# bayesiains/nflows

Measured on AMD Instinct MI355X. Metric: log_prob samples/sec (dim=64, K=8, 32-layer RQ-NSF) + max |fwd∘inv − x|, higher is better.
Workload: dtype f32 (inputs, outputs, spline arithmetic, accumulation; conditioner GEMMs: every fp32 operand carried as 3 f16 pieces = 33 significand bits, i.e. at the reference's own fp32 operand width, 5 cross products per multiply-add -- 3 on the f16 MFMA, the 2 at the 2^-22 level from the pieces' high bytes on

## Files before the change

### include/nflows_amd.h

```cpp
#ifndef NFLOWS_AMD_H
#define NFLOWS_AMD_H

#include <stddef.h>
#include <stdint.h>

#ifdef __cplusplus
extern "C" {
#endif

#define NFA_ABI_VERSION 16

#define NFA_OK 0
#define NFA_ERR_INVALID_ARGUMENT 1
#define NFA_ERR_UNSUPPORTED 2
#define NFA_ERR_MIN_BIN_WIDTH 3
#define NFA_ERR_MIN_BIN_HEIGHT 4
#define NFA_ERR_HIP 5

#define NFA_STATUS_OUTSIDE_DOMAIN 1
#define NFA_STATUS_NEG_DISCRIMINANT 2
#define NFA_STATUS_BAD_INDEX 4

#define NFA_FLAG_INVERSE 1
#define NFA_FLAG_ACCUMULATE_LOGABSDET 2
// ... 307 lines not shown
                                   const nfa_rqs_spec *spec, int32_t inverse, void *stream);
int nfa_quadratic_spline_backward_f32(const float *inputs, const float *unnormalized_widths,
                                      const float *unnormalized_heights, int32_t num_heights,
                                      const float *grad_outputs, const float *grad_logabsdet,
                                      float *grad_inputs, float *grad_unnormalized_widths,
                                      float *grad_unnormalized_heights, int64_t n,
                                      const nfa_rqs_spec *spec, int32_t inverse, void *stream);

int nfa_cubic_spline_backward_f32(const float *inputs, const float *unnormalized_widths,
                                  const float *unnormalized_heights,
                                  const float *unnorm_derivatives_left,
                                  const float *unnorm_derivatives_right, const float *grad_outputs,
                                  const float *grad_logabsdet, float *grad_inputs,
                                  float *grad_unnormalized_widths, float *grad_unnormalized_heights,
                                  float *grad_unnorm_derivatives_left,
                                  float *grad_unnorm_derivatives_right, int64_t n,
                                  const nfa_rqs_spec *spec, int32_t inverse, void *stream);

size_t nfa_linear_wgrad_workspace_bytes(int64_t batch, int32_t in_features, int32_t out_features);
int nfa_linear_wgrad_f32(const float *inputs, const float *grad_outputs, float *grad_weight,
                         float *grad_bias, void *workspace, int64_t batch, int32_t in_features,
                         int32_t out_features, int32_t flags, void *stream);

size_t nfa_linear_wgrad_batched_workspace_bytes(int32_t count, int64_t batch, int32_t in_features, int32_t out_features);
int nfa_linear_wgrad_batched_f32(int32_t count, const float *const *inputs, const float *const *grad_outputs,
                                 float *const *grad_weight, float *const *grad_bias, void *workspace, int64_t batch,
                                 int32_t in_features, int32_t out_features, int32_t flags, void *stream);

int nfa_profile_enable(int32_t max_launches);
int nfa_profile_collect(float *durations_ms, int32_t capacity, int32_t *count);

int nfa_last_layer_kernel(char *buffer, int32_t capacity);

void nfa_debug_k7_trace(void *device_buffer);

#ifdef __cplusplus
}
#endif
#endif
```

### nflows_amd/_native.py

```python
import ctypes
import os

import torch

_PKG_DIR = os.path.dirname(os.path.abspath(__file__))
LIB_PATH = os.environ.get("NFLOWS_AMD_LIB") or os.path.join(_PKG_DIR, "libnflows_amd.so")

OK = 0
ERR_INVALID_ARGUMENT = 1
ERR_UNSUPPORTED = 2
ERR_MIN_BIN_WIDTH = 3
ERR_MIN_BIN_HEIGHT = 4
ERR_HIP = 5

STATUS_OUTSIDE_DOMAIN = 1
STATUS_NEG_DISCRIMINANT = 2
STATUS_BAD_INDEX = 4

FLAG_INVERSE, FLAG_ACCUMULATE_LOGABSDET, FLAG_WEIGHTS_BF16X3, FLAG_LOGITS_LOG2E = 1, 2, 4, 8
FLAG_STANDARD_NORMAL_LOG_PROB, FLAG_SKIP_OUTPUTS = 16, 32
FLAG_RESIDUAL_BLOCKS = 64
FLAG_PAD_COLUMNS_SHIFT = 8
FLAG_ACTIVATION_SHIFT = 12
ACTIVATION_RELU, ACTIVATION_LEAKY_RELU, ACTIVATION_ELU, ACTIVATION_TANH = 0, 1, 2, 3
# ... 36 lines not shown
    "nfa_rqs_flow_resnet_context_redo_f32",
    "nfa_linear_spline_f32",
    "nfa_quadratic_spline_f32",
    "nfa_cubic_spline_f32",
    "nfa_linear_spline_backward_f32",
    "nfa_quadratic_spline_backward_f32",
    "nfa_cubic_spline_backward_f32",
    "nfa_rqs_elementwise_f32",
    "nfa_searchsorted_f32",
    "nfa_rqs_shared_f32",
    "nfa_affine_coupling_f32",
    "nfa_affine_autoregressive_f32",
    "nfa_permute_cols_b32",
    "nfa_lu_linear_f32",
    "nfa_lu_linear_backward_f32",
    "nfa_norm_workspace_bytes",
    "nfa_norm_slab_count",
    "nfa_norm_column_stats_f32",
    "nfa_norm_column_sums_f32",
    "nfa_norm_map_f32",
    "nfa_norm_map_backward_f32",
    "nfa_norm_batch_backward_f32",
    "nfa_rowsum_f32",
    "nfa_standard_normal_log_prob_f32",
    "nfa_sum_count_f64",
    "nfa_sum_count_workspace_bytes",
    "nfa_linear_wgrad_workspace_bytes",
    "nfa_linear_wgrad_f32",
    "nfa_linear_wgrad_batched_workspace_bytes",
    "nfa_linear_wgrad_batched_f32",
    "nfa_profile_enable",
    "nfa_profile_collect",
    "nfa_last_layer_kernel",
    "nfa_debug_k7_trace",
)


class NativeLibraryMissing(RuntimeError):
    pass


class NativeError(RuntimeError):
    def __init__(self, code, message):
        super().__init__("libnflows_amd: %s (code %d)" % (message, code))
        self.code = code


class RqsSpec(ctypes.Structure):

    _fields_ = [
        ("num_bins", ctypes.c_int32),
        ("tails", ctypes.c_int32),
        ("left", ctypes.c_double),
        ("right", ctypes.c_double),
        ("bottom", ctypes.c_double),
        ("top", ctypes.c_double),
        ("min_bin_width", ctypes.c_double),
        ("min_bin_height", ctypes.c_double),
        ("min_derivative", ctypes.c_double),
        ("softplus_beta", ctypes.c_double),
        ("tail_logit", ctypes.c_double),
        ("wh_divisor", ctypes.c_double),
    ]


_lib = None
# ... 101 lines not shown
    lib.nfa_norm_slab_count.argtypes = [i64, i32]
    lib.nfa_norm_column_stats_f32.restype = ctypes.c_int
    lib.nfa_norm_column_stats_f32.argtypes = [vp] * 5 + [i64, i32, vp]
    lib.nfa_norm_column_sums_f32.restype = ctypes.c_int
    lib.nfa_norm_column_sums_f32.argtypes = [vp] * 7 + [i64, i32, vp]
    lib.nfa_norm_map_f32.restype = ctypes.c_int
    lib.nfa_norm_map_f32.argtypes = [vp] * 10 + [i64, i32, ctypes.c_double, i32, i32, vp]
    lib.nfa_norm_map_backward_f32.restype = ctypes.c_int
    lib.nfa_norm_map_backward_f32.argtypes = [vp] * 9 + [i64, i32, ctypes.c_double, i32, i32, vp]
    lib.nfa_norm_batch_backward_f32.restype = ctypes.c_int
    lib.nfa_norm_batch_backward_f32.argtypes = [vp] * 7 + [i64, i32, vp]
    lib.nfa_rowsum_f32.restype = ctypes.c_int
    lib.nfa_rowsum_f32.argtypes = [vp, vp, i64, i64, vp]
    lib.nfa_standard_normal_log_prob_f32.restype = ctypes.c_int
    lib.nfa_standard_normal_log_prob_f32.argtypes = [vp, vp, vp, i64, i64, vp]
    lib.nfa_sum_count_f64.restype = ctypes.c_int
    lib.nfa_sum_count_f64.argtypes = [vp, i64, vp, vp, vp]
    lib.nfa_sum_count_workspace_bytes.restype = ctypes.c_size_t
    lib.nfa_sum_count_workspace_bytes.argtypes = []
    lib.nfa_linear_wgrad_workspace_bytes.restype = ctypes.c_size_t
    lib.nfa_linear_wgrad_workspace_bytes.argtypes = [i64, i32, i32]
    lib.nfa_linear_wgrad_f32.restype = ctypes.c_int
    lib.nfa_linear_wgrad_f32.argtypes = [vp, vp, vp, vp, vp, i64, i32, i32, i32, vp]
    lib.nfa_linear_wgrad_batched_workspace_bytes.restype = ctypes.c_size_t
    lib.nfa_linear_wgrad_batched_workspace_bytes.argtypes = [i32, i64, i32, i32]
    lib.nfa_linear_wgrad_batched_f32.restype = ctypes.c_int
    lib.nfa_linear_wgrad_batched_f32.argtypes = [i32, vp, vp, vp, vp, vp, i64, i32, i32, i32, vp]
    lib.nfa_profile_enable.restype = ctypes.c_int
    lib.nfa_profile_enable.argtypes = [i32]
    lib.nfa_profile_collect.restype = ctypes.c_int
    lib.nfa_profile_collect.argtypes = [ctypes.POINTER(ctypes.c_float), i32, ctypes.POINTER(i32)]
    lib.nfa_last_layer_kernel.restype = ctypes.c_int
    lib.nfa_last_layer_kernel.argtypes = [ctypes.c_char_p, i32]


def load():
    global _lib
    if _lib is None:
        if not os.path.exists(LIB_PATH):
            raise NativeLibraryMissing(
                "%s not found; nflows_amd has no fallback path. Build it with "
                "`make -C nflows_amd/csrc` (hipcc --offload-arch=gfx950)." % LIB_PATH
            )
        lib = ctypes.CDLL(LIB_PATH)
        missing = [name for name in EXPORTS if not hasattr(lib, name)]
        if missing:
            raise NativeLibraryMissing("%s lacks symbols: %s" % (LIB_PATH, ", ".join(missing)))
        _declare(lib)
        if lib.nfa_abi_version() != ABI_VERSION:
            raise NativeLibraryMissing("ABI version mismatch: library %d, binding %d"
                                       % (lib.nfa_abi_version(), ABI_VERSION))
        _lib = lib
    return _lib


def check(code):
    if code == OK:
        return
    lib = load()
    msg = lib.nfa_strerror(code).decode()
    if code in (ERR_MIN_BIN_WIDTH, ERR_MIN_BIN_HEIGHT):
        raise ValueError(msg)
    if code == ERR_HIP:
        msg += " (hipError_t %d)" % lib.nfa_last_hip_error()
    raise NativeError(code, msg)

# ... 31 lines not shown
```

### nflows_amd/csrc/launch_plan.hpp

```cpp
#pragma once

#include <stddef.h>
#include <stdint.h>

namespace nfa {

constexpr int kBlock = 256;
constexpr int kWave = 64;
constexpr int kDefaultDynLds = 64 * 1024;
constexpr int kCuLds = 160 * 1024;

inline int round_up4(int n) { return (n + 3) & ~3; }

inline bool aligned16(const void* p) { return (reinterpret_cast<uintptr_t>(p) & 15) == 0; }


inline int sample_rows(int lanes, int dt, int D, int64_t batch) {
    int R = dt > 0 ? lanes / dt : lanes / (D < lanes ? D : lanes);
    if (R < 1) R = 1;
    if ((int64_t)R > batch) R = (int)batch;
    return R;
}

struct SampleTile {
// ... 14 lines not shown
        t.C = (int)((budget - chunk_fixed) / ((size_t)P * 4));
        t.C = (t.C / kBlock) * kBlock;
        if (t.C >= dt) t.C = 0;
    }
    t.lds = (size_t)lds_floats(t.R, t.C) * 4;
    t.ok = t.lds <= budget && (int64_t)t.R * dt < 65536 && (int64_t)t.R * D < 65536;
    return t;
}

inline bool aligned_tile(int dt, int D, int P, int R, int64_t batch) {
    return dt > 0 && (dt * P) % 4 == 0 && D % 4 == 0 && R * dt <= kBlock && R * D <= 2 * kBlock && (int64_t)R <= batch;
}

inline int64_t full_rows(int64_t batch, int64_t rows_per_tile) { return (batch / rows_per_tile) * rows_per_tile; }

template <typename F>
inline int plan_element_tile(int floor, size_t budget, F&& bytes) {
    int T = kBlock;
    while (T > floor && (size_t)bytes(T) > budget) T >>= 1;
    return (size_t)bytes(T) <= budget ? T : 0;
}

inline int64_t persistent_grid(int cus, int per_cu, int64_t tiles) {
    const int64_t g = (int64_t)cus * per_cu;
    return g > tiles ? tiles : g;
}
inline int64_t persistent_grid(int cus, size_t lds, int cap, int64_t tiles) {
    int per_cu = (int)((size_t)kCuLds / (lds + 256));
    if (per_cu > cap) per_cu = cap;
    if (per_cu < 1) per_cu = 1;
    return persistent_grid(cus, per_cu, tiles);
}

}
```

### nflows_amd/csrc/rqs_resnet_f16x3.hip

```cpp

#include "rqs_resnet_f16x3_kernel.hpp"

using namespace nfa;

static k8x::KernelFn f16x3_kernel(bool inverse, int init_ks, int K, bool dbg) {
    if (K != 8) {
        const k8x::KernelFn kern = k8x::bins_kernel_a(K, inverse, init_ks);
        return kern ? kern : k8x::bins_kernel_b(K, inverse, init_ks);
    }
    if (init_ks == 4)
        return dbg ? (inverse ? k8x::rqs_resnet_f16x3_kernel<true, 4, true> : k8x::rqs_resnet_f16x3_kernel<false, 4, true>)
                   : (inverse ? k8x::rqs_resnet_f16x3_kernel<true, 4> : k8x::rqs_resnet_f16x3_kernel<false, 4>);
    return dbg ? (inverse ? k8x::rqs_resnet_f16x3_kernel<true, 2, true> : k8x::rqs_resnet_f16x3_kernel<false, 2, true>)
               : (inverse ? k8x::rqs_resnet_f16x3_kernel<true, 2> : k8x::rqs_resnet_f16x3_kernel<false, 2>);
}

static int launch_f16x3(const LayerCall& c, const float* scales, float act_scale, float* dbg_logits = nullptr) {
    int exponent = 0;
    if (!(act_scale > 0.0f) || frexpf(act_scale, &exponent) != 0.5f) return NFA_ERR_INVALID_ARGUMENT;
    k8x::Args a;
    int activation = 0;
    int rc = check_layer_call(c, {NFA_FLAG_ACTIVATION_MASK, true, false, false}, &a.sp, &activation);
    if (rc != NFA_OK) return rc;
    if (activation != NFA_ACTIVATION_RELU || (dbg_logits && a.sp.K != 8)) return NFA_ERR_UNSUPPORTED;
    if (c.batch == 0) return NFA_OK;
    if (!layer_buffers_given(c) || !c.bias || !scales || !c.redo) return NFA_ERR_INVALID_ARGUMENT;
    rc = fill_layer_args(a, c);
    if (rc != NFA_OK) return rc;
    a.act_scale = act_scale;
    a.bias = c.bias;
    a.scales = scales;
    a.tables = c.tables;
    a.redo = c.redo;
    a.dbg_logits = dbg_logits;
    const int init_ks = c.num_identity > 32 ? 4 : 2;
    const int rows_per_feature = spline_rows_per_feature(a.sp.K);
    a.num_stages = init_ks + 16 * c.num_blocks + 2 * (c.num_transform * rows_per_feature / 32);
    a.bias_per_layer = 128 + 256 * c.num_blocks + c.num_transform * rows_per_feature;
    const size_t lds = (size_t)kRing * kStageVec4 * 16 + (size_t)(kBlock / kWave) * c.features * kRowPad * sizeof(float) +
                       (size_t)c.num_transform * rows_per_feature * sizeof(float);
    int64_t blocks = c.batch >> 7;
    const int64_t per_cu = lds + 2048 <= 80 * 1024 ? 2 : 1;
    const int64_t cap = (int64_t)device_cu_count() * per_cu;
    if (blocks > cap) blocks = cap;
    const bool inv = (c.flags & NFA_FLAG_INVERSE) != 0;
    const k8x::KernelFn kern = f16x3_kernel(inv, init_ks, a.sp.K, dbg_logits);
    if (!kern) return NFA_ERR_UNSUPPORTED;
    note_layer_kernel("k8x::rqs_resnet_f16x3_kernel<inverse=%d, init_ks=%d, K=%d, dbg=%d>", inv ? 1 : 0, init_ks, a.sp.K, dbg_logits ? 1 : 0);
    return launch_kernel(kern, dim3((unsigned)blocks), dim3(kBlock), lds, (hipStream_t)c.stream, a, kCuLds - 2048);
}

extern "C" int nfa_rqs_flow_resnet_f16x3_f32(const float* inputs, const void* weights_packed, const float* bias_packed,
                                             const float* scales, const int32_t* flow_tables, int32_t num_layers,
                                             float* outputs, float* logabsdet, int32_t* redo_blocks, int32_t* status,
                                             int64_t batch, int32_t features, int32_t num_transform,
                                             int32_t num_identity, int32_t hidden_features, int32_t num_blocks,
                                             float act_scale, const nfa_rqs_spec* spec, int32_t flags, void* stream) {
    return launch_f16x3({inputs, weights_packed, bias_packed, flow_tables, num_layers, outputs, logabsdet, redo_blocks,
                         status, batch, features, num_transform, num_identity, hidden_features, num_blocks, spec, flags,
                         stream, nullptr, 0, 0},
                        scales, act_scale);
}

extern "C" int nfa_rqs_flow_resnet_f16x3_logits_f32(const float* inputs, const void* weights_packed,
                                                    const float* bias_packed, const float* scales,
                                                    const int32_t* flow_tables, int32_t num_layers, float* outputs,
                                                    float* logabsdet, int32_t* redo_blocks, int32_t* status,
                                                    int64_t batch, int32_t features, int32_t num_transform,
                                                    int32_t num_identity, int32_t hidden_features, int32_t num_blocks,
                                                    float act_scale, const nfa_rqs_spec* spec, int32_t flags,
                                                    void* stream, float* logits) {
    if (!logits) return NFA_ERR_INVALID_ARGUMENT;
    return launch_f16x3({inputs, weights_packed, bias_packed, flow_tables, num_layers, outputs, logabsdet, redo_blocks,
                         status, batch, features, num_transform, num_identity, hidden_features, num_blocks, spec, flags,
                         stream, nullptr, 0, 0},
                        scales, act_scale, logits);
}
```

### nflows_amd/ops.py

```python
import ctypes
import math
import os

import numpy as np
import torch

from . import _native as N
from . import autograd as AG
from .errors import InputOutsideDomain

_status_words = {}
_error_mode = "deferred"
_launch_hook = None


_last_redo = None


def last_redo_blocks():
    return None if _last_redo is None else int((_last_redo != 0).sum().item())


def set_launch_hook(hook):
    global _launch_hook
# ... 1887 lines not shown
    rows = logits_packed.shape[0]
    tiles = num_transform * 24 // 32
    v = logits_packed.view(rows, tiles, 2, 4, 4)
    packed_rows = v.permute(0, 1, 3, 2, 4).reshape(rows, tiles * 32)
    order = _k7_row_order(num_transform).to(logits_packed.device)
    out = torch.empty_like(packed_rows).index_copy_(1, order, packed_rows)
    return out.view(rows, num_transform, 24)[..., :23]


class capture_last_layer_logits:
    active = None

    def __enter__(self):
        self.logits = self.redo = None
        self.launches = 0
        capture_last_layer_logits.active = self
        return self

    def __exit__(self, *exc):
        capture_last_layer_logits.active = None
        return False

    def buffer(self, rows, num_transform, device):
        self._packed = torch.full((rows, num_transform * 24), float("nan"), dtype=torch.float32, device=device)
        self._dt = num_transform
        self.launches += 1
        return self._packed

    def finish(self, redo):
        self.logits = unpack_last_layer_logits(self._packed, self._dt)
        self.redo = redo


def rqs_coupling_resnet_f16x3(inputs, packed_f16x3, packed_exact, tables, num_transform, num_identity, num_blocks,
                              spec, inverse=False, accumulate_into=None, num_layers=1,
                              standard_normal_log_prob=False, pad=None, act_scale=K8X_ACT_SCALE):
    weights, biases, scales = packed_f16x3

    def launch(x, ctx, out, lad, redo, flags, status, stream):
        lib = N.load()
        B, D = x.shape
        args = (N.ptr(x), N.ptr(weights), N.ptr(biases), N.ptr(scales), N.ptr(tables), num_layers, N.ptr(out),
                N.ptr(lad), N.ptr(redo), status, B, D, num_transform, num_identity, 128, num_blocks,
                float(act_scale), ctypes.byref(spec), flags, stream)
        capture = capture_last_layer_logits.active
        if capture is None:
            return lib.nfa_rqs_flow_resnet_f16x3_f32(*args)
        rc = lib.nfa_rqs_flow_resnet_f16x3_logits_f32(*args, N.ptr(capture.buffer(B, num_transform, x.device)))
        if rc == N.OK:
            capture.finish(redo)
        return rc
    return _whole_layer_launch(launch, inputs, inverse, accumulate_into, standard_normal_log_prob, pad, spec=spec,
                               redo=(*packed_exact, tables, num_layers, num_transform, num_identity, num_blocks))


def rqs_coupling_fused_linear(inputs, hidden, weight_packed, bias_padded, transform_idx, spec,
                              inverse=False, in_perm=None, out_scatter=None, accumulate_into=None):
    N.require_device_f32("inputs", inputs, 2)
    N.require_device_f32("hidden", hidden, 2)
    dev = inputs.device
    B, D = inputs.shape
    tidx = _idx("transform_features", transform_idx, dev)
    perm = _idx("in_perm", in_perm, dev, D)
    scat = _idx("out_scatter", out_scatter, dev, D)
    x = inputs.detach().contiguous()
    h = hidden.detach().contiguous()
    out = torch.empty_like(x)
    lad, flags = _lad_buffer(accumulate_into, B, dev, inverse)
    if weight_packed.dtype == torch.bfloat16:
        flags |= N.FLAG_WEIGHTS_BF16X3
    with torch.cuda.device(dev):
        rc = N.load().nfa_rqs_coupling_fused_linear_f32(
            N.ptr(x), N.ptr(h), N.ptr(weight_packed), N.ptr(bias_padded), N.ptr(tidx), N.ptr(perm),
            N.ptr(scat), N.ptr(out), N.ptr(lad), N.ptr(_status_word(dev)), B, D, tidx.numel(),
            h.shape[1], ctypes.byref(spec), flags, N.stream_handle(dev))
    if rc == N.ERR_UNSUPPORTED:
        return None
    N.check(rc)
# ... 10 lines not shown
```

Before: 25.71 million.

## Add wide K8 kernel processing two row tiles per block sharing streamed weights

Adds a new persistent kernel variant for K=8 that processes two 128-row tiles per workgroup, so each streamed weight stage in the LDS ring feeds MFMAs for both tiles. Next-tile activation splitting is interleaved between the matrix ops. A deeper six-slot ring uses buffer-to-LDS loads. The wide path is chosen automatically when the batch yields at least two wide blocks per CU and its LDS need fits, with a runtime override. This halves per-row weight traffic and barrier cost, in exchange for higher register and LDS pressure and lower occupancy.

```diff
diff --git a/include/nflows_amd.h b/include/nflows_amd.h
--- a/include/nflows_amd.h
+++ b/include/nflows_amd.h
@@ -363,6 +363,9 @@
 
 int nfa_last_layer_kernel(char *buffer, int32_t capacity);
 
+int nfa_k8x_wide_override(int32_t mode, int32_t grid_cap);
+int nfa_k8x_wide_lds_bytes(int32_t features, int32_t num_transform);
+
 void nfa_debug_k7_trace(void *device_buffer);
 
 #ifdef __cplusplus
diff --git a/nflows_amd/_native.py b/nflows_amd/_native.py
--- a/nflows_amd/_native.py
+++ b/nflows_amd/_native.py
@@ -92,6 +92,8 @@
     "nfa_profile_enable",
     "nfa_profile_collect",
     "nfa_last_layer_kernel",
+    "nfa_k8x_wide_override",
+    "nfa_k8x_wide_lds_bytes",
     "nfa_debug_k7_trace",
 )
 
@@ -259,6 +261,10 @@
     lib.nfa_profile_collect.argtypes = [ctypes.POINTER(ctypes.c_float), i32, ctypes.POINTER(i32)]
     lib.nfa_last_layer_kernel.restype = ctypes.c_int
     lib.nfa_last_layer_kernel.argtypes = [ctypes.c_char_p, i32]
+    lib.nfa_k8x_wide_override.restype = ctypes.c_int
+    lib.nfa_k8x_wide_override.argtypes = [i32, i32]
+    lib.nfa_k8x_wide_lds_bytes.restype = ctypes.c_int
+    lib.nfa_k8x_wide_lds_bytes.argtypes = [i32, i32]
 
 
 def load():
diff --git a/nflows_amd/csrc/launch_plan.hpp b/nflows_amd/csrc/launch_plan.hpp
--- a/nflows_amd/csrc/launch_plan.hpp
+++ b/nflows_amd/csrc/launch_plan.hpp
@@ -70,4 +70,26 @@
     return persistent_grid(cus, per_cu, tiles);
 }
 
+constexpr int kWideStageBytes = 12 * 1024;
+constexpr int kWideRing = 6;
+constexpr int kWideRows = 256;
+
+inline size_t k8x_wide_lds(int D, int final_rows) {
+    return (size_t)kWideRing * kWideStageBytes + (size_t)8 * D * 33 * sizeof(float) + (size_t)final_rows * sizeof(float);
 }
+inline bool k8x_wide_fits(int D, int final_rows) { return k8x_wide_lds(D, final_rows) + 2048 <= (size_t)kCuLds; }
+
+inline int64_t k8x_wide_blocks(int64_t batch) { return ((batch >> 7) + 1) >> 1; }
+
+inline bool k8x_wide_selected(int64_t batch, int cus, int D, int final_rows, int mode) {
+    if (mode < 0 || !k8x_wide_fits(D, final_rows)) return false;
+    return mode > 0 || k8x_wide_blocks(batch) >= 2 * (int64_t)cus;
+}
+
+inline int64_t k8x_wide_grid(int64_t batch, int cus, int cap) {
+    int64_t g = persistent_grid(cus, 1, k8x_wide_blocks(batch));
+    if (cap > 0 && g > cap) g = cap;
+    return g;
+}
+
+}
diff --git a/nflows_amd/csrc/rqs_resnet_f16x3.hip b/nflows_amd/csrc/rqs_resnet_f16x3.hip
--- a/nflows_amd/csrc/rqs_resnet_f16x3.hip
+++ b/nflows_amd/csrc/rqs_resnet_f16x3.hip
@@ -1,7 +1,17 @@
 
 #include "rqs_resnet_f16x3_kernel.hpp"
 
+#include <atomic>
+
 using namespace nfa;
+
+namespace nfa {
+namespace k8x {
+KernelFn wide_kernel(bool inverse, int init_ks);
+}
+}
+
+static std::atomic<int> g_wide_mode{0}, g_wide_grid_cap{0};
 
 static k8x::KernelFn f16x3_kernel(bool inverse, int init_ks, int K, bool dbg) {
     if (K != 8) {
@@ -44,10 +54,30 @@
     const int64_t cap = (int64_t)device_cu_count() * per_cu;
     if (blocks > cap) blocks = cap;
     const bool inv = (c.flags & NFA_FLAG_INVERSE) != 0;
+    const int final_rows = c.num_transform * rows_per_feature;
+    if (a.sp.K == 8 && !dbg_logits &&
+        k8x_wide_selected(c.batch, device_cu_count(), c.features, final_rows, g_wide_mode.load(std::memory_order_relaxed))) {
+        const int64_t grid = k8x_wide_grid(c.batch, device_cu_count(), g_wide_grid_cap.load(std::memory_order_relaxed));
+        note_layer_kernel("k8x::rqs_resnet_f16x3_kernel_wide<inverse=%d, init_ks=%d, K=8>", inv ? 1 : 0, init_ks);
+        return launch_kernel(k8x::wide_kernel(inv, init_ks), dim3((unsigned)grid), dim3(kBlock),
+                             k8x_wide_lds(c.features, final_rows), (hipStream_t)c.stream, a, kCuLds - 2048);
+    }
     const k8x::KernelFn kern = f16x3_kernel(inv, init_ks, a.sp.K, dbg_logits);
     if (!kern) return NFA_ERR_UNSUPPORTED;
     note_layer_kernel("k8x::rqs_resnet_f16x3_kernel<inverse=%d, init_ks=%d, K=%d, dbg=%d>", inv ? 1 : 0, init_ks, a.sp.K, dbg_logits ? 1 : 0);
     return launch_kernel(kern, dim3((unsigned)blocks), dim3(kBlock), lds, (hipStream_t)c.stream, a, kCuLds - 2048);
+}
+
+extern "C" int nfa_k8x_wide_override(int32_t mode, int32_t grid_cap) {
+    if (grid_cap < 0) return NFA_ERR_INVALID_ARGUMENT;
+    g_wide_mode.store(mode < 0 ? -1 : (mode > 0 ? 1 : 0), std::memory_order_relaxed);
+    g_wide_grid_cap.store(grid_cap, std::memory_order_relaxed);
+    return NFA_OK;
+}
+
+extern "C" int nfa_k8x_wide_lds_bytes(int32_t features, int32_t num_transform) {
+    const int final_rows = num_transform * spline_rows_per_feature(8);
+    return k8x_wide_fits(features, final_rows) ? (int)k8x_wide_lds(features, final_rows) : 0;
 }
 
 extern "C" int nfa_rqs_flow_resnet_f16x3_f32(const float* inputs, const void* weights_packed, const float* bias_packed,
diff --git a/nflows_amd/csrc/rqs_resnet_f16x3_wide.hip b/nflows_amd/csrc/rqs_resnet_f16x3_wide.hip
--- /dev/null
+++ b/nflows_amd/csrc/rqs_resnet_f16x3_wide.hip
@@ -0,0 +1,13 @@
+
+#include "rqs_resnet_f16x3_wide_kernel.hpp"
+
+namespace nfa {
+namespace k8x {
+
+KernelFn wide_kernel(bool inverse, int init_ks) {
+    if (init_ks == 4) return inverse ? rqs_resnet_f16x3_kernel_wide<true, 4> : rqs_resnet_f16x3_kernel_wide<false, 4>;
+    return inverse ? rqs_resnet_f16x3_kernel_wide<true, 2> : rqs_resnet_f16x3_kernel_wide<false, 2>;
+}
+
+}
+}
diff --git a/nflows_amd/csrc/rqs_resnet_f16x3_wide_kernel.hpp b/nflows_amd/csrc/rqs_resnet_f16x3_wide_kernel.hpp
--- /dev/null
+++ b/nflows_amd/csrc/rqs_resnet_f16x3_wide_kernel.hpp
@@ -0,0 +1,611 @@
+#pragma once
+
+#include "launch_plan.hpp"
+#include "rqs_resnet_f16x3_kernel.hpp"
+
+namespace nfa {
+namespace k8x {
+namespace wide {
+
+constexpr int kRingW = kWideRing;
+static_assert(kWideStageBytes == kStageVec4 * 16, "launch_plan.hpp's stage size is the stream's");
+static_assert(kRingW >= 3 && 3 * (kRingW - 2) < 64, "the counted wait is a vmcnt immediate");
+
+__device__ __forceinline__ void request_stage_w(WeightStream& sm) {
+    const int dst_slot = sm.slot >= 1 ? sm.slot - 1 : kRingW - 1;
+    const char* stage = reinterpret_cast<const char*>(sm.w) + (size_t)sm.fetch * (kStageVec4 * 16);
+    const __amdgpu_buffer_rsrc_t rsrc =
+        __builtin_amdgcn_make_buffer_rsrc(const_cast<char*>(stage), (short)0, kStageVec4 * 16, 0x00020000);
+    const int wave = __builtin_amdgcn_readfirstlane(sm.tid >> 6);
+    char* slot = reinterpret_cast<char*>(sm.ring) + dst_slot * (kStageVec4 * 16) + wave * (kWave * 16);
+    const unsigned lane_off = (unsigned)(sm.tid & (kWave - 1)) * 16u;
+#pragma unroll
+    for (int i = 0; i < 3; ++i)
+        __builtin_amdgcn_raw_ptr_buffer_load_lds(rsrc, (__attribute__((address_space(3))) void*)(slot + i * kBlock * 16), 16,
+                                                 lane_off, i * kBlock * 16 + wave * (kWave * 16), 0, 0);
+    sm.fetch = (sm.fetch + 1 == sm.num_stages) ? 0 : sm.fetch + 1;
+}
+
+__device__ __forceinline__ void stream_advance_w(WeightStream& sm) {
+    asm volatile("s_waitcnt vmcnt(%0)\n\ts_waitcnt lgkmcnt(0)\n\ts_barrier" ::"n"(3 * (kRingW - 2)) : "memory");
+    sm.slot = (sm.slot + 1 == kRingW) ? 0 : sm.slot + 1;
+}
+
+struct Lead2 {
+    vec4f h0, l0;
+};
+__device__ __forceinline__ Lead2 read_lead2(const vec4f* stage) { return Lead2{stage[0 * 64], stage[1 * 64]}; }
+
+struct NoFill {
+    template <int G>
+    __device__ __forceinline__ void at() {}
+};
+
+__device__ __forceinline__ void split3_relu_head(float v0, float v1, float scale, unsigned& hi, float& t0, float& t1) {
+    NFA_K8X_ASM(
+        "v_maximum3_f32 %1, %3, 0, 0\n\t"
+        "v_maximum3_f32 %2, %4, 0, 0\n\t"
+        "v_fma_mixlo_f16 %0, %1, %5, 0 op_sel_hi:[0,0,0]\n\t"
+        "v_fma_mixhi_f16 %0, %2, %5, 0 op_sel_hi:[0,0,0]\n\t"
+        "v_fma_mix_f32 %1, %1, %5, -%0 op_sel_hi:[0,0,1]\n\t"
+        "v_fma_mix_f32 %2, %2, %5, -%0 op_sel:[0,0,1] op_sel_hi:[0,0,1]"
+        : "=&v"(hi), "=&v"(t0), "=&v"(t1)
+        : "v"(v0), "v"(v1), "s"(scale));
+}
+__device__ __forceinline__ void split3_tail(float& t0, float& t1, unsigned& lo, unsigned& rr) {
+    NFA_K8X_ASM(
+        "v_fma_mixlo_f16 %0, %2, 1.0, 0 op_sel_hi:[0,0,0]\n\t"
+        "v_fma_mixhi_f16 %0, %3, 1.0, 0 op_sel_hi:[0,0,0]\n\t"
+        "v_fma_mix_f32 %2, %2, 1.0, -%0 op_sel_hi:[0,0,1]\n\t"
+        "v_fma_mix_f32 %3, %3, 1.0, -%0 op_sel:[0,0,1] op_sel_hi:[0,0,1]\n\t"
+        "v_fma_mixlo_f16 %1, %2, %4, 0 op_sel_hi:[0,0,0]\n\t"
+        "v_fma_mixhi_f16 %1, %3, %4, 0 op_sel_hi:[0,0,0]"
+        : "=&v"(lo), "=&v"(rr), "+v"(t0), "+v"(t1)
+        : "s"(256.0f));
+}
+
+struct ReluFill {
+    const f32x16& sa;
+    const f32x16& sb;
+    float scale;
+    Pieces (&na)[2];
+    Pieces (&nb)[2];
+    i32x8& xa;
+    i32x8& xb;
+    float t0[2], t1[2];
+    unsigned hh[2];
+
+    template <int G>
+    __device__ __forceinline__ void at() {
+        constexpr int tile = G & 1;
+        const f32x16& s = tile ? sb : sa;
+        Pieces(&n)[2] = tile ? nb : na;
+        if constexpr (G < 32) {
+            constexpr int q2 = G >> 2;
+            if constexpr (((G >> 1) & 1) == 0) {
+                split3_relu_head(s[q2 * 2], s[q2 * 2 + 1], scale, hh[tile], t0[tile], t1[tile]);
+            } else {
+                unsigned lo, rr;
+                split3_tail(t0[tile], t1[tile], lo, rr);
+                n[q2 >> 2].h[q2 & 3] = hh[tile];
+                n[q2 >> 2].l[q2 & 3] = lo;
+                n[q2 >> 2].r[q2 & 3] = rr;
+            }
+        } else if constexpr (G < 36) {
+            constexpr unsigned kHigh = 0x07050301u;
+            constexpr int ks = (G >> 1) & 1;
+            i32x8& x = tile ? xb : xa;
+            const Pieces& p = n[ks];
+            x[ks * 4 + 0] = (int)__builtin_amdgcn_perm(p.r[1], p.r[0], kHigh);
+            x[ks * 4 + 1] = (int)__builtin_amdgcn_perm(p.r[3], p.r[2], kHigh);
+            x[ks * 4 + 2] = (int)__builtin_amdgcn_perm(p.h[1], p.h[0], kHigh);
+            x[ks * 4 + 3] = (int)__builtin_amdgcn_perm(p.h[3], p.h[2], kHigh);
+        }
+    }
+};
+
+#define NFA_K8XW_F16(G, ACCA, ACCB, A_, BA_, BB_)                           \
+    ACCA = NFA_K8X_F16(A_, BA_, ACCA);                                      \
+    NFA_K8X_FENCE();                                                        \
+    fill.template at<(G)>();                                                \
+    NFA_K8X_FENCE();                                                        \
+    ACCB = NFA_K8X_F16(A_, BB_, ACCB);                                      \
+    NFA_K8X_FENCE();                                                        \
+    fill.template at<(G) + 1>();                                            \
+    NFA_K8X_FENCE()
+#define NFA_K8XW_BF8(G, ACCA, ACCB, A_, BA_, BB_)                           \
+    ACCA = NFA_K8X_BF8(A_, BA_, ACCA);                                      \
+    NFA_K8X_FENCE();                                                        \
+    fill.template at<(G)>();                                                \
+    NFA_K8X_FENCE();                                                        \
+    ACCB = NFA_K8X_BF8(A_, BB_, ACCB);                                      \
+    NFA_K8X_FENCE();                                                        \
+    fill.template at<(G) + 1>();                                            \
+    NFA_K8X_FENCE()
+
+template <bool LAST, int G0, class Fill>
+__device__ __forceinline__ void stage_kmajor2(f32x16& a0, f32x16& a1, f32x16& c0, f32x16& c1, const Pieces (&pa)[2],
+                                              const i32x8& xa, const Pieces (&pb)[2], const i32x8& xb, WeightStream& sm, int lane,
+                                              Lead2& lead, Fill& fill) {
+    request_stage_w(sm);
+    const vec4f* cur = sm.ring + sm.slot * kStageVec4 + lane;
+    const f16x8 ah0_ = __builtin_bit_cast(f16x8, pa[0].h), al0_ = __builtin_bit_cast(f16x8, pa[0].l);
+    const f16x8 ah1_ = __builtin_bit_cast(f16x8, pa[1].h), al1_ = __builtin_bit_cast(f16x8, pa[1].l);
+    const f16x8 ch0_ = __builtin_bit_cast(f16x8, pb[0].h), cl0_ = __builtin_bit_cast(f16x8, pb[0].l);
+    const f16x8 ch1_ = __builtin_bit_cast(f16x8, pb[1].h), cl1_ = __builtin_bit_cast(f16x8, pb[1].l);
+    const vec4f lh1 = cur[2 * 64], ll1 = cur[3 * 64], x0l = cur[4 * 64], x0h = cur[5 * 64];
+    vec4f h0, l0, h1, l1, x1l, x1h;
+    NFA_K8X_FENCE();
+    {
+        const f16x8 wh0 = __builtin_bit_cast(f16x8, lead.h0), wl0 = __builtin_bit_cast(f16x8, lead.l0);
+        const f16x8 wh1 = __builtin_bit_cast(f16x8, lh1), wl1 = __builtin_bit_cast(f16x8, ll1);
+        const i32x8 wx = join_x(x0l, x0h);
+        NFA_K8XW_F16(G0 + 0, a0, c0, wh0, al0_, cl0_);
+        NFA_K8XW_F16(G0 + 2, a0, c0, wl0, ah0_, ch0_);
+        NFA_K8XW_F16(G0 + 4, a0, c0, wh0, ah0_, ch0_);
+        h0 = cur[6 * 64];
+        l0 = cur[7 * 64];
+        h1 = cur[8 * 64];
+        l1 = cur[9 * 64];
+        x1l = cur[10 * 64];
+        x1h = cur[11 * 64];
+        NFA_K8X_FENCE();
+        NFA_K8XW_F16(G0 + 6, a0, c0, wh1, al1_, cl1_);
+        NFA_K8XW_F16(G0 + 8, a0, c0, wl1, ah1_, ch1_);
+        NFA_K8XW_F16(G0 + 10, a0, c0, wh1, ah1_, ch1_);
+        NFA_K8XW_BF8(G0 + 12, a0, c0, wx, xa, xb);
+    }
+    const f16x8 wh0 = __builtin_bit_cast(f16x8, h0), wl0 = __builtin_bit_cast(f16x8, l0);
+    const f16x8 wh1 = __builtin_bit_cast(f16x8, h1), wl1 = __builtin_bit_cast(f16x8, l1);
+    const i32x8 wx = join_x(x1l, x1h);
+    NFA_K8XW_F16(G0 + 14, a1, c1, wh0, al0_, cl0_);
+    NFA_K8XW_F16(G0 + 16, a1, c1, wl0, ah0_, ch0_);
+    NFA_K8XW_F16(G0 + 18, a1, c1, wh0, ah0_, ch0_);
+    stream_advance_w(sm);
+    if constexpr (!LAST) lead = read_lead2(sm.ring + sm.slot * kStageVec4 + lane);
+    NFA_K8X_FENCE();
+    NFA_K8XW_F16(G0 + 20, a1, c1, wh1, al1_, cl1_);
+    NFA_K8XW_F16(G0 + 22, a1, c1, wl1, ah1_, ch1_);
+    NFA_K8XW_F16(G0 + 24, a1, c1, wh1, ah1_, ch1_);
+    NFA_K8XW_BF8(G0 + 26, a1, c1, wx, xa, xb);
+}
+
+template <int NKS>
+__device__ __forceinline__ void gemm_kmajor2(f32x16 (&accA)[4], f32x16 (&accB)[4], const Pieces (&pA)[8], const Pieces (&pB)[8],
+                                             WeightStream& sm, int lane) {
+    static_assert(NKS % 2 == 0, "pairs of k-steps");
+    Lead2 lead = read_lead2(sm.ring + sm.slot * kStageVec4 + lane);
+    NoFill fill;
+#pragma unroll
+    for (int pr = 0; pr < NKS / 2; ++pr) {
+        const Pieces a[2] = {pA[2 * pr], pA[2 * pr + 1]}, c[2] = {pB[2 * pr], pB[2 * pr + 1]};
+        const i32x8 xa = bf8_operand(a[0], a[1]), xb = bf8_operand(c[0], c[1]);
+        stage_kmajor2<false, 0>(accA[0], accA[1], accB[0], accB[1], a, xa, c, xb, sm, lane, lead, fill);
+        if (pr + 1 < NKS / 2) stage_kmajor2<false, 28>(accA[2], accA[3], accB[2], accB[3], a, xa, c, xb, sm, lane, lead, fill);
+        else stage_kmajor2<true, 28>(accA[2], accA[3], accB[2], accB[3], a, xa, c, xb, sm, lane, lead, fill);
+    }
+}
+
+template <int PR>
+__device__ __forceinline__ void relu_pairs2(f32x16 (&accA)[4], f32x16 (&accB)[4], const f32x16 (&srcA)[4], const f32x16 (&srcB)[4],
+                                            float scale, const Pieces (&a)[2], const i32x8& xa, const Pieces (&c)[2],
+                                            const i32x8& xb, WeightStream& sm, int lane, Lead2& lead) {
+    if constexpr (PR < 3) {
+        Pieces na[2], nc[2];
+        i32x8 nxa, nxb;
+        ReluFill fill{srcA[PR + 1], srcB[PR + 1], scale, na, nc, nxa, nxb, {0.0f, 0.0f}, {0.0f, 0.0f}, {0u, 0u}};
+        stage_kmajor2<false, 0>(accA[0], accA[1], accB[0], accB[1], a, xa, c, xb, sm, lane, lead, fill);
+        stage_kmajor2<false, 28>(accA[2], accA[3], accB[2], accB[3], a, xa, c, xb, sm, lane, lead, fill);
+        relu_pairs2<PR + 1>(accA, accB, srcA, srcB, scale, na, nxa, nc, nxb, sm, lane, lead);
+    } else {
+        NoFill fill;
+        stage_kmajor2<false, 0>(accA[0], accA[1], accB[0], accB[1], a, xa, c, xb, sm, lane, lead, fill);
+        stage_kmajor2<true, 28>(accA[2], accA[3], accB[2], accB[3], a, xa, c, xb, sm, lane, lead, fill);
+    }
+}
+__device__ __forceinline__ void gemm_kmajor_relu2(f32x16 (&accA)[4], f32x16 (&accB)[4], const f32x16 (&srcA)[4],
+                                                  const f32x16 (&srcB)[4], float scale, WeightStream& sm, int lane) {
+    Lead2 lead = read_lead2(sm.ring + sm.slot * kStageVec4 + lane);
+    Pieces a[2], c[2];
+    tile_to_pieces<true, true>(srcA[0], scale, a[0], a[1]);
+    tile_to_pieces<true, false>(srcB[0], scale, c[0], c[1]);
+    const i32x8 xa = bf8_operand(a[0], a[1]), xb = bf8_operand(c[0], c[1]);
+    relu_pairs2<0>(accA, accB, srcA, srcB, scale, a, xa, c, xb, sm, lane, lead);
+}
+#undef NFA_K8XW_F16
+#undef NFA_K8XW_BF8
+
+#define NFA_K8XW_PUMP_F16(U, A_, BA_, BB_)                                  \
+    accA = NFA_K8X_F16(A_, BA_, accA);                                      \
+    NFA_K8X_FENCE();                                                        \
+    wa.template span<(U), (U) + 1>();                                       \
+    NFA_K8X_FENCE();                                                        \
+    accB = NFA_K8X_F16(A_, BB_, accB);                                      \
+    NFA_K8X_FENCE();                                                        \
+    wb.template span<(U), (U) + 1>();                                       \
+    NFA_K8X_FENCE()
+#define NFA_K8XW_PUMP_BF8(U, A_, BA_, BB_)                                  \
+    accA = NFA_K8X_BF8(A_, BA_, accA);                                      \
+    NFA_K8X_FENCE();                                                        \
+    wa.template span<(U), (U) + 2>();                                       \
+    NFA_K8X_FENCE();                                                        \
+    accB = NFA_K8X_BF8(A_, BB_, accB);                                      \
+    NFA_K8X_FENCE();                                                        \
+    wb.template span<(U), (U) + 2>();                                       \
+    NFA_K8X_FENCE()
+
+template <int HS, class WA, class WB>
+__device__ __forceinline__ void stage_pumped2(f32x16& accA, f32x16& accB, const Pieces (&pA)[8], const i32x8 (&bxA)[4],
+                                              const Pieces (&pB)[8], const i32x8 (&bxB)[4], WeightStream& sm, int lane, Lead2& lead,
+                                              WA& wa, WB& wb) {
+    request_stage_w(sm);
+    const vec4f* cur = sm.ring + sm.slot * kStageVec4 + lane;
+    vec4f xa = cur[8 * 64], xb = cur[9 * 64];
+    vec4f fh0 = lead.h0, fl0 = lead.l0, fh1 = cur[2 * 64], fl1 = cur[3 * 64];
+    {
+        const f16x8 ah0_ = __builtin_bit_cast(f16x8, pA[HS * 4 + 0].h), al0_ = __builtin_bit_cast(f16x8, pA[HS * 4 + 0].l);
+        const f16x8 ah1_ = __builtin_bit_cast(f16x8, pA[HS * 4 + 1].h), al1_ = __builtin_bit_cast(f16x8, pA[HS * 4 + 1].l);
+        const f16x8 ch0_ = __builtin_bit_cast(f16x8, pB[HS * 4 + 0].h), cl0_ = __builtin_bit_cast(f16x8, pB[HS * 4 + 0].l);
+        const f16x8 ch1_ = __builtin_bit_cast(f16x8, pB[HS * 4 + 1].h), cl1_ = __builtin_bit_cast(f16x8, pB[HS * 4 + 1].l);
+        const f16x8 wh0 = __builtin_bit_cast(f16x8, fh0), wl0 = __builtin_bit_cast(f16x8, fl0);
+        const f16x8 wh1 = __builtin_bit_cast(f16x8, fh1), wl1 = __builtin_bit_cast(f16x8, fl1);
+        const i32x8 wx = join_x(xa, xb);
+        NFA_K8XW_PUMP_F16(HS * 16 + 0, wh0, al0_, cl0_);
+        NFA_K8XW_PUMP_F16(HS * 16 + 1, wl0, ah0_, ch0_);
+        NFA_K8XW_PUMP_F16(HS * 16 + 2, wh0, ah0_, ch0_);
+        fh0 = cur[4 * 64];
+        fl0 = cur[5 * 64];
+        NFA_K8XW_PUMP_F16(HS * 16 + 3, wh1, al1_, cl1_);
+        NFA_K8XW_PUMP_F16(HS * 16 + 4, wl1, ah1_, ch1_);
+        NFA_K8XW_PUMP_F16(HS * 16 + 5, wh1, ah1_, ch1_);
+        fh1 = cur[6 * 64];
+        fl1 = cur[7 * 64];
+        NFA_K8XW_PUMP_BF8(HS * 16 + 6, wx, bxA[HS * 2 + 0], bxB[HS * 2 + 0]);
+        xa = cur[10 * 64];
+        xb = cur[11 * 64];
+    }
+    {
+        const f16x8 ah0_ = __builtin_bit_cast(f16x8, pA[HS * 4 + 2].h), al0_ = __builtin_bit_cast(f16x8, pA[HS * 4 + 2].l);
+        const f16x8 ah1_ = __builtin_bit_cast(f16x8, pA[HS * 4 + 3].h), al1_ = __builtin_bit_cast(f16x8, pA[HS * 4 + 3].l);
+        const f16x8 ch0_ = __builtin_bit_cast(f16x8, pB[HS * 4 + 2].h), cl0_ = __builtin_bit_cast(f16x8, pB[HS * 4 + 2].l);
+        const f16x8 ch1_ = __builtin_bit_cast(f16x8, pB[HS * 4 + 3].h), cl1_ = __builtin_bit_cast(f16x8, pB[HS * 4 + 3].l);
+        const f16x8 wh0 = __builtin_bit_cast(f16x8, fh0), wl0 = __builtin_bit_cast(f16x8, fl0);
+        const f16x8 wh1 = __builtin_bit_cast(f16x8, fh1), wl1 = __builtin_bit_cast(f16x8, fl1);
+        const i32x8 wx = join_x(xa, xb);
+        NFA_K8XW_PUMP_F16(HS * 16 + 8, wh0, al0_, cl0_);
+        NFA_K8XW_PUMP_F16(HS * 16 + 9, wl0, ah0_, ch0_);
+        NFA_K8XW_PUMP_F16(HS * 16 + 10, wh0, ah0_, ch0_);
+        NFA_K8XW_PUMP_F16(HS * 16 + 11, wh1, al1_, cl1_);
+        NFA_K8XW_PUMP_F16(HS * 16 + 12, wl1, ah1_, ch1_);
+        NFA_K8XW_PUMP_F16(HS * 16 + 13, wh1, ah1_, ch1_);
+        stream_advance_w(sm);
+        lead = read_lead2(sm.ring + sm.slot * kStageVec4 + lane);
+        NFA_K8X_FENCE();
+        NFA_K8XW_PUMP_BF8(HS * 16 + 14, wx, bxA[HS * 2 + 1], bxB[HS * 2 + 1]);
+    }
+}
+#undef NFA_K8XW_PUMP_F16
+#undef NFA_K8XW_PUMP_BF8
+
+template <class WA, class WB>
+__device__ __forceinline__ void gemm_tile_pumped2(f32x16& accA, f32x16& accB, const Pieces (&pA)[8], const i32x8 (&bxA)[4],
+                                                  const Pieces (&pB)[8], const i32x8 (&bxB)[4], WeightStream& sm, int lane,
+                                                  Lead2& lead, WA&& wa, WB&& wb) {
+    stage_pumped2<0>(accA, accB, pA, bxA, pB, bxB, sm, lane, lead, wa, wb);
+    stage_pumped2<1>(accA, accB, pA, bxA, pB, bxB, sm, lane, lead, wa, wb);
+}
+
+}
+
+template <bool INVERSE, int INIT_KS>
+__global__ void __launch_bounds__(kBlock, 1) rqs_resnet_f16x3_kernel_wide(const Args a) {
+    using namespace wide;
+    constexpr int kFinalRows = 24;
+    constexpr int NW = kBlock / kWave;
+    extern __shared__ __attribute__((aligned(16))) float lds_dyn[];
+    __shared__ int s_tab[2][kTabLayer];
+    __shared__ int s_final[128];
+    __shared__ int s_bad[2][NW];
+    const int tid = threadIdx.x, lane = tid & 63, wave = __builtin_amdgcn_readfirstlane(tid >> 6);
+    const int D = a.D, dt = a.dt;
+    int my_status = 0;
+    auto checked = [&](int v, bool used) {
+        my_status |= (used && (v < 0 || v >= D)) ? NFA_STATUS_BAD_INDEX : 0;
+        return v < 0 ? 0 : (v >= D ? D - 1 : v);
+    };
+    const int te = tid & (kTabLayer - 1);
+    s_tab[0][te] = checked(a.tables[te], te < kTabTr ? te < a.di : te - kTabTr < dt);
+    s_final[te] = checked(a.tables[a.num_layers * kTabLayer + te], te < D);
+
+    WeightStream sm;
+    sm.w = a.w;
+    sm.ring = reinterpret_cast<vec4f*>(lds_dyn);
+    sm.fetch = 0;
+    sm.num_stages = a.num_stages * a.num_layers;
+    sm.tid = tid;
+#pragma unroll
+    for (int s = 0; s < kRingW - 1; ++s) {
+        sm.slot = s + 1 == kRingW ? 0 : s + 1;
+        request_stage_w(sm);
+    }
+    sm.slot = 0;
+    asm volatile("s_waitcnt vmcnt(0)" ::: "memory");
+    __syncthreads();
+
+    lds_f32* s_rows = (lds_f32*)lds_dyn + kRingW * kStageVec4 * 4 + wave * 2 * D * kRowPad;
+    lds_f32* s_fbias = (lds_f32*)lds_dyn + kRingW * kStageVec4 * 4 + NW * 2 * D * kRowPad;
+    const int groups = dt >> 2;
+    const int64_t num_quads = a.batch >> 7;
+    const int64_t num_wide = (num_quads + 1) >> 1;
+    const int gemms = 2 + 2 * a.num_blocks;
+    const float S = a.act_scale;
+    int tb = 0;
+
+    for (int64_t wb_ = blockIdx.x; wb_ < num_wide; wb_ += gridDim.x) {
+        const bool second = 2 * wb_ + 1 < num_quads;
+        int lane_here = lane, di = a.di;
+        asm volatile("" : "+v"(lane_here), "+s"(di));
+        const int half = lane_here >> 5, r = lane_here & 31;
+        lds_f32* s_row[2] = {s_rows, s_rows + D * kRowPad};
+        int64_t row0[2];
+#pragma unroll
+        for (int t = 0; t < 2; ++t) {
+            row0[t] = ((2 * wb_ + t) << 7) + (wave << 5);
+            const bool live = t == 0 || second;
+            const vec4f* xv = reinterpret_cast<const vec4f*>(a.x + (live ? row0[t] : 0) * D);
+            const int nvec = D * 8;
+            for (int e0 = lane; e0 < nvec; e0 += kWave * 4) {
+                vec4f v[4];
+#pragma unroll
+                for (int u = 0; u < 4; ++u) {
+                    const int e = e0 + u * kWave;
+                    v[u] = live ? xv[e < nvec ? e : 0] : vec4f{0.0f, 0.0f, 0.0f, 0.0f};
+                }
+#pragma unroll
+                for (int u = 0; u < 4; ++u) {
+                    const int e = e0 + u * kWave;
+                    if (e < nvec) {
+                        const int rr = (e * 4) / D, c0 = e * 4 - rr * D;
+                        s_row[t][(c0 + 0) * kRowPad + rr] = v[u].x;
+                        s_row[t][(c0 + 1) * kRowPad + rr] = v[u].y;
+                        s_row[t][(c0 + 2) * kRowPad + rr] = v[u].z;
+                        s_row[t][(c0 + 3) * kRowPad + rr] = v[u].w;
+                    }
+                }
+            }
+        }
+        __builtin_amdgcn_fence(__ATOMIC_RELEASE, "wavefront");
+        __builtin_amdgcn_fence(__ATOMIC_ACQUIRE, "wavefront");
+
+        float lad_acc[2] = {0.0f, 0.0f};
+        int quad_status[2] = {0, 0};
+        for (int layer = 0; layer < a.num_layers; ++layer) {
+            const int* tab = s_tab[tb];
+            {
+                unsigned all = ~0u;
+                asm volatile("" : "+s"(all));
+                const int te_l = (int)__builtin_amdgcn_mbcnt_hi(all, __builtin_amdgcn_mbcnt_lo(all, 0u)) + ((wave & 1) << 6);
+                const int nl = layer + 1 < a.num_layers ? layer + 1 : 0;
+                s_tab[tb ^ 1][te_l] = checked(a.tables[nl * kTabLayer + te_l], te_l < kTabTr ? te_l < a.di : te_l - kTabTr < dt);
+            }
+            const float* bias = a.bias + (size_t)layer * a.bias_per_layer;
+            const int bh = half * 16;
+            const float* sc = a.scales + (size_t)layer * gemms * 2;
+            Pieces p[2][8];
+
+#pragma unroll
+            for (int t = 0; t < 2; ++t) {
+#pragma unroll
+                for (int ks = 0; ks < INIT_KS; ++ks) {
+#pragma unroll
+                    for (int j2 = 0; j2 < 4; ++j2) {
+                        const int i0 = ks * 16 + half * 8 + j2 * 2;
+                        float v0 = s_row[t][tab[kTabId + i0] * kRowPad + r], v1 = s_row[t][tab[kTabId + i0 + 1] * kRowPad + r];
+                        v0 = i0 < di ? v0 : 0.0f;
+                        v1 = i0 + 1 < di ? v1 : 0.0f;
+                        unsigned hi, lo, rr;
+                        split3_scaled(v0, v1, S, hi, lo, rr);
+                        p[t][ks].h[j2] = hi;
+                        p[t][ks].l[j2] = lo;
+                        p[t][ks].r[j2] = rr;
+                    }
+                }
+            }
+
+            f32x16 h[2][4];
+            float hs;
+            {
+#pragma unroll
+                for (int t = 0; t < 4; ++t) {
+                    load_bias_tile(h[0][t], bias + t * 32 + bh);
+                    h[1][t] = h[0][t];
+                }
+                gemm_kmajor2<INIT_KS>(h[0], h[1], p[0], p[1], sm, lane);
+                float s0[2];
+                uniform_load(sc, s0);
+                hs = s0[0];
+            }
+            bias += 128;
+            sc += 2;
+            {
+                const float* fbias = a.bias + (size_t)layer * a.bias_per_layer + 128 + 256 * a.num_blocks;
+                for (int i = tid; i < dt * kFinalRows; i += kBlock) s_fbias[i] = fbias[i];
+                if (a.num_blocks == 0) __syncthreads();
+            }
+
+            for (int blk = 0; blk < a.num_blocks; ++blk) {
+                float sb[4];
+                f32x16 u[2][4];
+#pragma unroll
+                for (int t = 0; t < 4; ++t) {
+                    load_bias_tile(u[0][t], bias + t * 32 + bh);
+                    u[1][t] = u[0][t];
+                }
+                gemm_kmajor_relu2(u[0], u[1], h[0], h[1], hs, sm, lane);
+                uniform_load(sc, sb);
+                const float skip = hs * sb[3];
+#pragma unroll
+                for (int t = 0; t < 4; ++t) {
+                    f32x16 b1;
+                    load_bias_tile(b1, bias + 128 + t * 32 + bh);
+#pragma unroll
+                    for (int q_ = 0; q_ < 16; ++q_) {
+                        h[0][t][q_] = __builtin_fmaf(h[0][t][q_], skip, b1[q_]);
+                        h[1][t][q_] = __builtin_fmaf(h[1][t][q_], skip, b1[q_]);
+                    }
+                }
+                gemm_kmajor_relu2(h[0], h[1], u[0], u[1], sb[0], sm, lane);
+                hs = sb[2];
+                bias += 256;
+                sc += 4;
+            }
+
+#pragma unroll
+            for (int t2 = 0; t2 < 2; ++t2) {
+#pragma unroll
+                for (int t = 0; t < 4; ++t) {
+                    if (t2 == 0 && t == 0) tile_to_pieces<false, true>(h[t2][t], hs, p[t2][2 * t], p[t2][2 * t + 1]);
+                    else tile_to_pieces<false, false>(h[t2][t], hs, p[t2][2 * t], p[t2][2 * t + 1]);
+                }
+            }
+
+            {
+                using Steps = FusedSteps<INVERSE, 8>;
+                Steps fa[2] = {Steps{}, Steps{}}, fb[2] = {Steps{}, Steps{}};
+                float sf[2];
+                uniform_load(sc, sf);
+                const float kappa = sf[0];
+#pragma unroll
+                for (int t = 0; t < 2; ++t) {
+                    fa[t].kappa = fb[t].kappa = kappa;
+                    fa[t].kl2e = fb[t].kl2e = 1.44269502162933349609375f * kappa;
+                    fa[t].tail_s = fb[t].tail_s = a.sp.tail_logit * sf[1];
+                }
+                int off_b = 0;
+                const lds_f32* fbias = s_fbias + half * 16;
+                i32x8 bx[2][4];
+#pragma unroll
+                for (int t = 0; t < 2; ++t)
+#pragma unroll
+                    for (int j = 0; j < 4; ++j) bx[t][j] = bf8_operand(p[t][2 * j], p[t][2 * j + 1]);
+                Lead2 lead = read_lead2(sm.ring + sm.slot * kStageVec4 + lane);
+                f32x16 acc[2][3];
+                auto commit = [&](int t, Steps& f, lds_f32* slot) {
+                    *slot = f.y;
+                    lad_acc[t] += f.lad;
+                    quad_status[t] |= f.status;
+                };
+                UnitWeave<k8h::kUnitNumA, Steps> w0a{fa[0], fb[0], a.sp}, w0b{fa[1], fb[1], a.sp};
+                UnitWeave<k8h::kUnitFinishA, Steps> w1a{fa[0], fb[0], a.sp}, w1b{fa[1], fb[1], a.sp};
+                UnitWeave<k8h::kUnitFinishB, Steps> w2a{fa[0], fb[0], a.sp}, w2b{fa[1], fb[1], a.sp};
+                for (int g = 0; g < groups; ++g) {
+                    const int off0 = tab[kTabTr + g * 4 + half * 2] * kRowPad + r;
+                    const int off1 = tab[kTabTr + g * 4 + half * 2 + 1] * kRowPad + r;
+                    load_bias_tile(acc[0][0], fbias + (g * 3 + 0) * 32);
+                    acc[1][0] = acc[0][0];
+                    if (g > 0) {
+                        gemm_tile_pumped2(acc[0][0], acc[1][0], p[0], bx[0], p[1], bx[1], sm, lane, lead, w2a, w2b);
+                        commit(0, fb[0], s_row[0] + off_b);
+                        commit(1, fb[1], s_row[1] + off_b);
+                    } else {
+                        gemm_tile_pumped2(acc[0][0], acc[1][0], p[0], bx[0], p[1], bx[1], sm, lane, lead, NoWeave{}, NoWeave{});
+                    }
+#pragma unroll
+                    for (int t = 0; t < 2; ++t) {
+                        fa[t].x = s_row[t][off0];
+#pragma unroll
+                        for (int j = 0; j < 8; ++j) {
+                            fa[t].ew[j] = acc[t][0][j];
+                            fa[t].eh[j] = acc[t][0][8 + j];
+                        }
+                    }
+                    load_bias_tile(acc[0][1], fbias + (g * 3 + 1) * 32);
+                    acc[1][1] = acc[0][1];
+                    gemm_tile_pumped2(acc[0][1], acc[1][1], p[0], bx[0], p[1], bx[1], sm, lane, lead, w0a, w0b);
+#pragma unroll
+                    for (int t = 0; t < 2; ++t) {
+                        fb[t].x = s_row[t][off1];
+#pragma unroll
+                        for (int j = 0; j < 8; ++j) {
+                            if (j < 7) fa[t].sd[j] = acc[t][1][j];
+                            fb[t].ew[j] = acc[t][1][8 + j];
+                        }
+                    }
+                    load_bias_tile(acc[0][2], fbias + (g * 3 + 2) * 32);
+                    acc[1][2] = acc[0][2];
+                    gemm_tile_pumped2(acc[0][2], acc[1][2], p[0], bx[0], p[1], bx[1], sm, lane, lead, w1a, w1b);
+#pragma unroll
+                    for (int t = 0; t < 2; ++t) {
+                        commit(t, fa[t], s_row[t] + off0);
+#pragma unroll
+                        for (int j = 0; j < 8; ++j) {
+                            fb[t].eh[j] = acc[t][2][j];
+                            if (j < 7) fb[t].sd[j] = acc[t][2][8 + j];
+                        }
+                    }
+                    off_b = off1;
+                }
+#pragma unroll
+                for (int t = 0; t < 2; ++t) {
+                    k8h::spline_unit_range<k8h::kUnitFinishB, 0, k8h::spline_unit_slices<k8h::kUnitFinishB, Steps>()>(fa[t], fb[t], a.sp);
+                    commit(t, fb[t], s_row[t] + off_b);
+                }
+            }
+            tb ^= 1;
+            __builtin_amdgcn_fence(__ATOMIC_RELEASE, "wavefront");
+            __builtin_amdgcn_fence(__ATOMIC_ACQUIRE, "wavefront");
+        }
+
+        bool wave_bad[2];
+        float sumsq[2];
+#pragma unroll
+        for (int t = 0; t < 2; ++t) {
+            lad_acc[t] += __shfl_xor(lad_acc[t], 32, kWave);
+            sumsq[t] = tile_row_sumsq((const float*)s_row[t], a.Ds, half, r);
+            const bool bad = not_finite(lad_acc[t]) || not_finite(sumsq[t]);
+            wave_bad[t] = __builtin_amdgcn_ballot_w64(bad) != 0;
+            if (lane == 0) s_bad[t][wave] = wave_bad[t] ? 1 : 0;
+        }
+        asm volatile("s_waitcnt vmcnt(0)" ::: "memory");
+        __syncthreads();
+#pragma unroll
+        for (int t = 0; t < 2; ++t) {
+            if (t == 1 && !second) break;
+            int any_bad = 0;
+#pragma unroll
+            for (int w_ = 0; w_ < NW; ++w_) any_bad |= s_bad[t][w_];
+            if (!any_bad) {
+                if (!a.skip_out) {
+                    vec4f* ov = reinterpret_cast<vec4f*>(a.out + row0[t] * D);
+                    const int nvec = D * 8;
+                    for (int e = lane; e < nvec; e += kWave) {
+                        const int rr = (e * 4) / D, c0 = e * 4 - rr * D;
+                        vec4f v;
+                        v.x = s_row[t][s_final[c0 + 0] * kRowPad + rr];
+                        v.y = s_row[t][s_final[c0 + 1] * kRowPad + rr];
+                        v.z = s_row[t][s_final[c0 + 2] * kRowPad + rr];
+                        v.w = s_row[t][s_final[c0 + 3] * kRowPad + rr];
+                        ov[e] = v;
+                    }
+                }
+                if (half == 0) {
+                    float* dst = a.lad + row0[t] + r;
+                    float v = a.accumulate ? *dst + lad_acc[t] : lad_acc[t];
+                    if (a.normal) v = (-0.5f * sumsq[t] - a.log_z) + v;
+                    *dst = v;
+                }
+                my_status |= quad_status[t];
+            }
+            if (tid == 0) a.redo[2 * wb_ + t] = any_bad ? 1 : 0;
+        }
+        asm volatile("s_waitcnt vmcnt(0)" ::: "memory");
+        __syncthreads();
+    }
+    asm volatile("s_waitcnt vmcnt(0)" ::: "memory");
+    if (my_status && a.status) atomicOr(a.status, my_status);
+}
+
+KernelFn wide_kernel(bool inverse, int init_ks);
+
+}
+}
diff --git a/nflows_amd/ops.py b/nflows_amd/ops.py
--- a/nflows_amd/ops.py
+++ b/nflows_amd/ops.py
@@ -1943,6 +1943,19 @@
         self.redo = redo
 
 
+K8X_WIDE = None
+K8X_WIDE_GRID_CAP = 0
+_k8x_wide_sent = (None, 0)
+
+
+def _send_k8x_wide(lib):
+    global _k8x_wide_sent
+    want = (K8X_WIDE, int(K8X_WIDE_GRID_CAP))
+    if want != _k8x_wide_sent:
+        N.check(lib.nfa_k8x_wide_override(0 if want[0] is None else (1 if want[0] else -1), want[1]))
+        _k8x_wide_sent = want
+
+
 def rqs_coupling_resnet_f16x3(inputs, packed_f16x3, packed_exact, tables, num_transform, num_identity, num_blocks,
                               spec, inverse=False, accumulate_into=None, num_layers=1,
                               standard_normal_log_prob=False, pad=None, act_scale=K8X_ACT_SCALE):
@@ -1955,6 +1968,7 @@
                 N.ptr(lad), N.ptr(redo), status, B, D, num_transform, num_identity, 128, num_blocks,
                 float(act_scale), ctypes.byref(spec), flags, stream)
         capture = capture_last_layer_logits.active
+        _send_k8x_wide(lib)
         if capture is None:
             return lib.nfa_rqs_flow_resnet_f16x3_f32(*args)
         rc = lib.nfa_rqs_flow_resnet_f16x3_logits_f32(*args, N.ptr(capture.buffer(B, num_transform, x.device)))
```

Result: slower. 24.33 million (-5.4%).
